# dyollb/segmantic

Hardware: AMD Instinct MI355X
Metric: 3D UNet train voxels/s on 128^3 bf16 (higher is better)
Workload: dtype bf16

## Files before the change

segmantic_amd/csrc/conv_fwd_impl.h:

```cpp
#pragma once
#include "common.h"
#include "fin_tail.h"

namespace segmi {

struct ConvParams {
  const void* in;
  void* out;
  const void* wfrag;
  const float* bias;
  const float* alpha;
  const void* res;
  float* stats;
  int N, Di, Hi, Wi, Do, Ho, Wo, Cin, Cout, ldi, ldo, ldr;
  int tz, ty, tx;
  int nchunks, ntiles_total;
  const float* in_scale;
  const float* in_shift;
  const float* in_alpha;
  int act_tiles;
  int stats_tiles;
  const float* bias2;
  const void* bx;
  int ldbx;
  const float* bmean; const float* binvstd; const float* bgamma; const float* bbeta; const float* balpha;
  float* bpart;
  int fin_on;
  FinTail ft;
  BnFin bfin;
  BnBwdFin bbfin;
  int xcd;
};

template <typename T, int CK, int KS, int S, int TD, int TH, int TW>
struct ConvGeom {
  static constexpr int KG = Elem<T>::KG;
  static constexpr int SPT = CK / KG;
  static constexpr int NTAPS = KS * KS * KS;
  static constexpr int NSLOT = NTAPS * SPT;
  static constexpr int NSTEP = (NSLOT + 3) / 4;
  static constexpr int PAD = (KS - 1) / 2;
  static constexpr int HD = (TD - 1) * S + KS;
  static constexpr int HH = (TH - 1) * S + KS;
  static constexpr int HW = (TW - 1) * S + KS;
  static constexpr int RAWB = CK * (int)sizeof(T);
  static constexpr int ROWB = RAWB == 32 ? 32 : RAWB + 16;
  static constexpr int CPR = RAWB / 16;
  static constexpr int NVT = TD * TH * TW / 16;
  static constexpr int VTW = NVT / 4;
  static constexpr int LDS_BYTES = HD * HH * HW * ROWB;
  static_assert(NVT % 4 == 0, "tile must give each wave whole voxel tiles");
  static_assert(SPT == 2 || SPT == 4 || SPT == 8, "unsupported chunk width");
};

template <typename T, int CK, int KS, int S, int NT, int TD, int TH, int TW>
__global__ __launch_bounds__(256) void conv_fwd_mfma_kernel(ConvParams p) {
  using G = ConvGeom<T, CK, KS, S, TD, TH, TW>;
  extern __shared__ __attribute__((aligned(16))) char smem[];
  const int tid = threadIdx.x, lane = tid & 63, wave = tid >> 6;
  const int g = lane >> 4, r = lane & 15;

  int t = blockIdx.x;
  const int txi = t % p.tx; t /= p.tx;
  const int tyi = t % p.ty; t /= p.ty;
  const int tzi = t % p.tz;
  const int n = t / p.tz;
  const int oz0 = tzi * TD, oy0 = tyi * TH, ox0 = txi * TW;
  const int iz0 = oz0 * S - G::PAD, iy0 = oy0 * S - G::PAD, ix0 = ox0 * S - G::PAD;
  const int nt0 = blockIdx.y * NT;

  f32x4 acc[G::VTW][NT];
#pragma unroll
  for (int i = 0; i < G::VTW; ++i)
#pragma unroll
    for (int j = 0; j < NT; ++j) acc[i][j] = f32x4{0.f, 0.f, 0.f, 0.f};

  int vaddr[G::VTW];
#pragma unroll
  for (int i = 0; i < G::VTW; ++i) {
    const int idx = (wave * G::VTW + i) * 16 + r;
    const int x = idx % TW, y = (idx / TW) % TH, z = idx / (TW * TH);
    vaddr[i] = ((z * S * G::HH + y * S) * G::HW + x * S) * G::ROWB;
  }

  constexpr bool PRE = G::NSTEP * NT <= 16;
  constexpr int WD = NT <= 2 ? (G::NSTEP < 4 ? G::NSTEP : 4) : 2;
  constexpr int NCH = G::HD * G::HH * G::HW * G::CPR;
  constexpr int NLD = (NCH + 255) / 256;
  constexpr bool PF = (G::VTW * NT * 4 + NLD * 4) <= 160;
  const char* inb = (const char*)p.in;
  frag_t stg[PF ? NLD : 1];
  auto fetch = [&](int c) {
#pragma unroll
    for (int k = 0; k < NLD; ++k) {
      const int i = tid + 256 * k;
      const int v = i / G::CPR, ch = i % G::CPR;
      const int hx = v % G::HW, hy = (v / G::HW) % G::HH, hz = v / (G::HW * G::HH);
      const int z = iz0 + hz, y = iy0 + hy, x = ix0 + hx;
      frag_t val = frag_t{0u, 0u, 0u, 0u};
      if (i < NCH && (unsigned)z < (unsigned)p.Di && (unsigned)y < (unsigned)p.Hi &&
          (unsigned)x < (unsigned)p.Wi) {
        const int64_t e = ((((int64_t)n * p.Di + z) * p.Hi + y) * p.Wi + x) * p.ldi + c * CK;
        val = *reinterpret_cast<const frag_t*>(inb + e * (int64_t)sizeof(T) + ch * 16);
      }
      if constexpr (PF) stg[k] = val;
      else if (i < NCH) *reinterpret_cast<frag_t*>(smem + v * G::ROWB + ch * 16) = val;
    }
  };
  if constexpr (PF) fetch(0);
  for (int c = 0; c < p.nchunks; ++c) {
    if (c > 0) __syncthreads();
    const char* wb = (const char*)p.wfrag +
                     (((int64_t)c * G::NSTEP) * p.ntiles_total + nt0) * 1024 + lane * 16;
    frag_t wall[PRE ? G::NSTEP : 1][NT];
    frag_t wq[PRE ? 1 : WD][NT];
    if constexpr (PRE) {
#pragma unroll
      for (int s = 0; s < G::NSTEP; ++s)
#pragma unroll
        for (int j = 0; j < NT; ++j)
          wall[s][j] = *reinterpret_cast<const frag_t*>(wb + ((int64_t)s * p.ntiles_total + j) * 1024);
    } else {
#pragma unroll
      for (int s = 0; s < WD; ++s)
#pragma unroll
        for (int j = 0; j < NT; ++j)
          wq[s][j] = *reinterpret_cast<const frag_t*>(wb + ((int64_t)s * p.ntiles_total + j) * 1024);
    }
    if constexpr (PF) {
#pragma unroll
      for (int k = 0; k < NLD; ++k) {
        const int i = tid + 256 * k;
        if (i < NCH) *reinterpret_cast<frag_t*>(smem + (i / G::CPR) * G::ROWB + (i % G::CPR) * 16) = stg[k];
      }
    } else {
      fetch(c);
    }
    __syncthreads();
    if constexpr (PF) {
      if (c + 1 < p.nchunks) fetch(c + 1);
    }
#pragma unroll
    for (int s = 0; s < G::NSTEP; ++s) {
      int loff;
      if constexpr (G::SPT == 2) {
        const int t0 = 2 * s, t1 = 2 * s + 1;
        const int o0 = ((t0 / (KS * KS)) * G::HH + (t0 / KS) % KS) * G::HW + t0 % KS;
        const int o1 = t1 < G::NTAPS
                           ? ((t1 / (KS * KS)) * G::HH + (t1 / KS) % KS) * G::HW + t1 % KS
                           : 0;
        loff = ((g >> 1) ? o1 : o0) * G::ROWB + (g & 1) * 16;
      } else {
        const int tap = (4 * s) / G::SPT;
        const int sub0 = (4 * s) % G::SPT;
        const int o0 = ((tap / (KS * KS)) * G::HH + (tap / KS) % KS) * G::HW + tap % KS;
        loff = o0 * G::ROWB + (sub0 + g) * 16;
      }
      frag_t wf[NT];
      if constexpr (PRE) {
#pragma unroll
        for (int j = 0; j < NT; ++j) wf[j] = wall[s][j];
      } else {
#pragma unroll
        for (int j = 0; j < NT; ++j) wf[j] = wq[s % WD][j];
        if (s + WD < G::NSTEP) {
#pragma unroll
          for (int j = 0; j < NT; ++j)
            wq[s % WD][j] = *reinterpret_cast<const frag_t*>(
                wb + ((int64_t)(s + WD) * p.ntiles_total + j) * 1024);
        }
      }
#pragma unroll
      for (int i = 0; i < G::VTW; ++i) {
        const frag_t a = *reinterpret_cast<const frag_t*>(smem + vaddr[i] + loff);
#pragma unroll
        for (int j = 0; j < NT; ++j) acc[i][j] = mma16<T>(wf[j], a, acc[i][j]);
      }
    }
  }

  f32x4 bias4[NT];
#pragma unroll
  for (int j = 0; j < NT; ++j) {
    bias4[j] = f32x4{0.f, 0.f, 0.f, 0.f};
    if (p.bias2 && nt0 + j >= p.act_tiles)
      bias4[j] = *reinterpret_cast<const f32x4*>(p.bias2 + (nt0 + j - p.act_tiles) * 16 + 4 * g);
    else if (p.bias) bias4[j] = *reinterpret_cast<const f32x4*>(p.bias + (nt0 + j) * 16 + 4 * g);
  }
  const bool has_alpha = p.alpha != nullptr;
  const float alpha = has_alpha ? *p.alpha : 0.f;
  const bool do_stats = p.stats != nullptr && (p.stats_tiles == 0 || nt0 < p.stats_tiles);
  const int stats_c = p.stats_tiles > 0 ? 16 * p.stats_tiles : p.Cout;
  f32x4 ssum[NT], ssq[NT];
#pragma unroll
  for (int j = 0; j < NT; ++j) {
    ssum[j] = f32x4{0.f, 0.f, 0.f, 0.f};
    ssq[j] = f32x4{0.f, 0.f, 0.f, 0.f};
  }
  T* outp = (T*)p.out;
  const T* resp = (const T*)p.res;
  f32x4 resv[G::VTW][NT];
  if (resp) {
#pragma unroll
    for (int i = 0; i < G::VTW; ++i) {
      const int idx = (wave * G::VTW + i) * 16 + r;
      const int oz = oz0 + idx / (TW * TH), oy = oy0 + (idx / TW) % TH, ox = ox0 + idx % TW;
      const bool valid = oz < p.Do && oy < p.Ho && ox < p.Wo;
      const int64_t vox = (((int64_t)n * p.Do + oz) * p.Ho + oy) * p.Wo + ox;
#pragma unroll
      for (int j = 0; j < NT; ++j)
        resv[i][j] = valid ? load4<T>(resp + vox * p.ldr + (nt0 + j) * 16 + 4 * g)
                           : f32x4{0.f, 0.f, 0.f, 0.f};
    }
#pragma unroll
    for (int i = 0; i < G::VTW; ++i)
#pragma unroll
      for (int j = 0; j < NT; ++j) touch_v(resv[i][j]);
  }
#pragma unroll
  for (int j = 0; j < NT; ++j) touch_v(bias4[j]);
  if constexpr (PF) {
#pragma unroll
    for (int k = 0; k < NLD; ++k) touch_v(stg[k]);
  }
#pragma unroll
  for (int i = 0; i < G::VTW; ++i) {
    const int idx = (wave * G::VTW + i) * 16 + r;
    const int oz = oz0 + idx / (TW * TH), oy = oy0 + (idx / TW) % TH, ox = ox0 + idx % TW;
    const bool valid = oz < p.Do && oy < p.Ho && ox < p.Wo;
    const int64_t vox = (((int64_t)n * p.Do + oz) * p.Ho + oy) * p.Wo + ox;
#pragma unroll
    for (int j = 0; j < NT; ++j) {
      f32x4 v = acc[i][j] + bias4[j];
      if (valid) {
        if (do_stats && (p.stats_tiles == 0 || nt0 + j < p.stats_tiles)) {
          ssum[j] += v;
          ssq[j] += v * v;
        }
        if (has_alpha && (p.act_tiles == 0 || nt0 + j < p.act_tiles)) {
#pragma unroll
          for (int e = 0; e < 4; ++e) v[e] = v[e] > 0.f ? v[e] : alpha * v[e];
        }
        const int co = (nt0 + j) * 16 + 4 * g;
        if (resp) v += resv[i][j];
        store4<T>(outp + vox * p.ldo + co, v);
      }
    }
  }
  if (do_stats) {
    __syncthreads();
    float* red = reinterpret_cast<float*>(smem);
#pragma unroll
    for (int j = 0; j < NT; ++j)
#pragma unroll
      for (int e = 0; e < 4; ++e) {
        const float a = row16_sum(ssum[j][e]);
        const float b = row16_sum(ssq[j][e]);
        if (r == 0) {
          red[(wave * 2 + 0) * NT * 16 + j * 16 + 4 * g + e] = a;
          red[(wave * 2 + 1) * NT * 16 + j * 16 + 4 * g + e] = b;
        }
      }
    __syncthreads();
    if (tid < 2 * NT * 16) {
      const int which = tid / (NT * 16), ch = tid % (NT * 16);
      float sacc = 0.f;
#pragma unroll
      for (int w = 0; w < 4; ++w) sacc += red[(w * 2 + which) * NT * 16 + ch];
      if (nt0 * 16 + ch < stats_c)
        fin_store(&p.stats[((int64_t)blockIdx.x * 2 + which) * stats_c + nt0 * 16 + ch], sacc);
    }
    fin_tail_run<BnFin, 256, offsetof(ConvParams, ft), offsetof(ConvParams, bfin)>(p.stats, smem);
  }
}

template <typename T, int CK, int KS, int S, int NT, int TD, int TH, int TW>
static int launch_conv_cfg(ConvParams p, hipStream_t st) {
  using G = ConvGeom<T, CK, KS, S, TD, TH, TW>;
  p.tz = cdiv(p.Do, TD);
  p.ty = cdiv(p.Ho, TH);
  p.tx = cdiv(p.Wo, TW);
  const int64_t nb = (int64_t)p.N * p.tz * p.ty * p.tx;
  SEGMI_CHECK_ARG(nb < (1ll << 31), "conv3d: too many tiles");
  dim3 grid((unsigned)nb, (unsigned)(p.Cout / (16 * NT)));
  constexpr int lds0 = G::LDS_BYTES > 4 * 2 * NT * 16 * 4 ? G::LDS_BYTES : 4 * 2 * NT * 16 * 4;
  p.fin_on = p.fin_on && p.stats;
  const int stats_c = p.stats_tiles > 0 ? 16 * p.stats_tiles : p.Cout;
  const dim3 sgrid(grid.x, (unsigned)cdiv(stats_c / 16, NT));
  const int lds = (int)fin_tail_arm(p, sgrid, 256, 2 * stats_c, lds0);
  auto kern = conv_fwd_mfma_kernel<T, CK, KS, S, NT, TD, TH, TW>;
  static bool attr_done = false;
  if (!attr_done && lds > 64 * 1024) {
    (void)hipFuncSetAttribute(reinterpret_cast<const void*>(kern),
                        hipFuncAttributeMaxDynamicSharedMemorySize, lds);
    attr_done = true;
  }
  hipLaunchKernelGGL(kern, grid, 256, lds, st, p);
  SEGMI_LAUNCH_CHECK("conv3d_fwd(mfma)");
  return SEGMI_OK;
}

template <typename T, int CK, int KS, int S, int NT>
static int launch_conv_tiles(const ConvParams& p, hipStream_t st) {
  const bool wide = p.Wo > 8;
  if constexpr (S == 1) {
    if (wide) return launch_conv_cfg<T, CK, KS, S, NT, 4, 8, 16>(p, st);
    return launch_conv_cfg<T, CK, KS, S, NT, 4, 4, 8>(p, st);
  } else {
    if (wide) return launch_conv_cfg<T, CK, KS, S, NT, 2, 4, 16>(p, st);
    return launch_conv_cfg<T, CK, KS, S, NT, 2, 4, 8>(p, st);
  }
}

template <typename T, int CK, int KS, int S>
static int launch_conv_nt(const ConvParams& p, hipStream_t st) {
  const int nt = p.Cout / 16;
  const bool wide = p.Wo > 8;
  const int td = S == 1 ? 4 : 2, th = S == 1 ? (wide ? 8 : 4) : 4, tw = wide ? 16 : 8;
  const int64_t tiles = (int64_t)p.N * cdiv(p.Do, td) * cdiv(p.Ho, th) * cdiv(p.Wo, tw);
  int sel = nt % 4 == 0 ? 4 : (nt % 2 == 0 ? 2 : 1);
  while (sel > 1 && tiles * (nt / sel) < 512) sel /= 2;
  if (sel == 4) return launch_conv_tiles<T, CK, KS, S, 4>(p, st);
  if (sel == 2) return launch_conv_tiles<T, CK, KS, S, 2>(p, st);
  return launch_conv_tiles<T, CK, KS, S, 1>(p, st);
}

template <typename T>
static int launch_conv_mfma_t(const ConvParams& p, int ksize, int stride, hipStream_t st) {
  constexpr int dt = DtypeOf<T>::value;
  const int ck = pick_ck(dt, p.Cin);
  if constexpr (sizeof(T) == 2) {
    if (ck == 32) {
      if (ksize == 3 && stride == 1) return launch_conv_nt<T, 32, 3, 1>(p, st);
      if (ksize == 3 && stride == 2) return launch_conv_nt<T, 32, 3, 2>(p, st);
      if (ksize == 1 && stride == 1) return launch_conv_nt<T, 32, 1, 1>(p, st);
    }
  }
  if (ksize == 3 && stride == 1) return launch_conv_nt<T, 16, 3, 1>(p, st);
  if (ksize == 3 && stride == 2) return launch_conv_nt<T, 16, 3, 2>(p, st);
  if (ksize == 1 && stride == 1) return launch_conv_nt<T, 16, 1, 1>(p, st);
  SEGMI_UNSUPPORTED("conv3d: unsupported ksize/stride %d/%d", ksize, stride);
}

static inline int conv_mfma_rows(const segmi_act* out, int stride) {
  const bool wide = out->w > 8;
  int td, th, tw;
  if (stride == 1) { td = 4; th = wide ? 8 : 4; tw = wide ? 16 : 8; }
  else { td = 2; th = 4; tw = wide ? 16 : 8; }
  return out->n * cdiv(out->d, td) * cdiv(out->h, th) * cdiv(out->w, tw);
}

}
```

segmantic_amd/csrc/conv_ks_impl.h:

```cpp
#pragma once
#include "conv_fwd_impl.h"

namespace segmi {

template <typename T, int CK, int KS, int S, int NT, int TD, int TH, int TW>
__global__ __launch_bounds__(256) void conv_fwd_ks_kernel(ConvParams p) {
  using G = ConvGeom<T, CK, KS, S, TD, TH, TW>;
  static_assert(G::SPT == 4, "k-split kernel: one k-step per tap");
  static_assert(G::NVT == 8, "k-split kernel: 8 voxel tiles per workgroup");
  constexpr int NSW = (G::NSTEP + 3) / 4;
  extern __shared__ __attribute__((aligned(16))) char smem[];
  const int tid = threadIdx.x, lane = tid & 63;
  const int wave = __builtin_amdgcn_readfirstlane(tid >> 6);
  const int g = lane >> 4, r = lane & 15;

  int t = blockIdx.x;
  const int txi = t % p.tx; t /= p.tx;
  const int tyi = t % p.ty; t /= p.ty;
  const int tzi = t % p.tz;
  const int n = t / p.tz;
  const int oz0 = tzi * TD, oy0 = tyi * TH, ox0 = txi * TW;
  const int iz0 = oz0 * S - G::PAD, iy0 = oy0 * S - G::PAD, ix0 = ox0 * S - G::PAD;
  const int nt0 = blockIdx.y * NT;

  f32x4 acc[8][NT];
#pragma unroll
  for (int i = 0; i < 8; ++i)
#pragma unroll
    for (int j = 0; j < NT; ++j) acc[i][j] = f32x4{0.f, 0.f, 0.f, 0.f};

  int vaddr[8];
#pragma unroll
  for (int i = 0; i < 8; ++i) {
    const int idx = i * 16 + r;
    const int x = idx % TW, y = (idx / TW) % TH, z = idx / (TW * TH);
    vaddr[i] = ((z * S * G::HH + y * S) * G::HW + x * S) * G::ROWB + g * 16;
  }
  int tapoff[NSW];
#pragma unroll
  for (int si = 0; si < NSW; ++si) {
    int tap = wave + 4 * si;
    if (tap > G::NTAPS - 1) tap = G::NTAPS - 1;
    tapoff[si] = (((tap / (KS * KS)) * G::HH + (tap / KS) % KS) * G::HW + tap % KS) * G::ROWB;
  }

  constexpr int NCH = G::HD * G::HH * G::HW * G::CPR;
  constexpr int NLD = (NCH + 255) / 256;
  const char* inb = (const char*)p.in;
  frag_t stg[NLD];
  auto fetch = [&](int c) {
#pragma unroll
    for (int k = 0; k < NLD; ++k) {
      const int i = tid + 256 * k;
      const int v = i / G::CPR, ch = i % G::CPR;
      const int hx = v % G::HW, hy = (v / G::HW) % G::HH, hz = v / (G::HW * G::HH);
      const int z = iz0 + hz, y = iy0 + hy, x = ix0 + hx;
      stg[k] = frag_t{0u, 0u, 0u, 0u};
      if (i < NCH && (unsigned)z < (unsigned)p.Di && (unsigned)y < (unsigned)p.Hi &&
          (unsigned)x < (unsigned)p.Wi) {
        const int64_t e = ((((int64_t)n * p.Di + z) * p.Hi + y) * p.Wi + x) * p.ldi + c * CK;
        stg[k] = *reinterpret_cast<const frag_t*>(inb + e * (int64_t)sizeof(T) + ch * 16);
      }
    }
  };
  const char* wb0 = (const char*)p.wfrag + (int64_t)nt0 * 1024 + lane * 16;
  frag_t wcur[NSW][NT], wnxt[NSW][NT];
  auto fetch_w = [&](int c, frag_t (&dst)[NSW][NT]) {
#pragma unroll
    for (int si = 0; si < NSW; ++si) {
      int s = wave + 4 * si;
      if (s > G::NSTEP - 1) s = G::NSTEP - 1;
#pragma unroll
      for (int j = 0; j < NT; ++j)
        dst[si][j] = *reinterpret_cast<const frag_t*>(
            wb0 + (((int64_t)c * G::NSTEP + s) * p.ntiles_total + j) * 1024);
    }
  };
  fetch(0);
  fetch_w(0, wcur);
  for (int c = 0; c < p.nchunks; ++c) {
    if (c > 0) __syncthreads();
#pragma unroll
    for (int k = 0; k < NLD; ++k) {
      const int i = tid + 256 * k;
      if (i < NCH) *reinterpret_cast<frag_t*>(smem + (i / G::CPR) * G::ROWB + (i % G::CPR) * 16) = stg[k];
    }
    __syncthreads();
    if (c + 1 < p.nchunks) {
      fetch(c + 1);
      fetch_w(c + 1, wnxt);
    }
#pragma unroll
    for (int si = 0; si < NSW; ++si) {
      const int s = wave + 4 * si;
      if (s < G::NSTEP) {
#pragma unroll
        for (int i = 0; i < 8; ++i) {
          const frag_t a = *reinterpret_cast<const frag_t*>(smem + vaddr[i] + tapoff[si]);
#pragma unroll
          for (int j = 0; j < NT; ++j) acc[i][j] = mma16<T>(wcur[si][j], a, acc[i][j]);
        }
      }
    }
#pragma unroll
    for (int si = 0; si < NSW; ++si)
#pragma unroll
      for (int j = 0; j < NT; ++j) wcur[si][j] = wnxt[si][j];
  }

  __syncthreads();
  f32x4* red = reinterpret_cast<f32x4*>(smem);
#pragma unroll
  for (int i = 0; i < 8; ++i)
#pragma unroll
    for (int j = 0; j < NT; ++j) red[((wave * 8 + i) * NT + j) * 64 + lane] = acc[i][j];
  __syncthreads();
  f32x4 fin[2][NT];
#pragma unroll
  for (int ii = 0; ii < 2; ++ii)
#pragma unroll
    for (int j = 0; j < NT; ++j) {
      const int i = wave * 2 + ii;
      f32x4 v = red[((0 * 8 + i) * NT + j) * 64 + lane];
      v += red[((1 * 8 + i) * NT + j) * 64 + lane];
      v += red[((2 * 8 + i) * NT + j) * 64 + lane];
      v += red[((3 * 8 + i) * NT + j) * 64 + lane];
      fin[ii][j] = v;
    }

  f32x4 bias4[NT];
#pragma unroll
  for (int j = 0; j < NT; ++j) {
    bias4[j] = f32x4{0.f, 0.f, 0.f, 0.f};
    if (p.bias) bias4[j] = *reinterpret_cast<const f32x4*>(p.bias + (nt0 + j) * 16 + 4 * g);
  }
  const bool has_alpha = p.alpha != nullptr;
  const float alpha = has_alpha ? *p.alpha : 0.f;
  f32x4 ssum[NT], ssq[NT];
#pragma unroll
  for (int j = 0; j < NT; ++j) {
    ssum[j] = f32x4{0.f, 0.f, 0.f, 0.f};
    ssq[j] = f32x4{0.f, 0.f, 0.f, 0.f};
  }
  T* outp = (T*)p.out;
  const T* resp = (const T*)p.res;
  f32x4 resv[2][NT];
  if (resp) {
#pragma unroll
    for (int ii = 0; ii < 2; ++ii) {
      const int idx = (wave * 2 + ii) * 16 + r;
      const int oz = oz0 + idx / (TW * TH), oy = oy0 + (idx / TW) % TH, ox = ox0 + idx % TW;
      const bool valid = oz < p.Do && oy < p.Ho && ox < p.Wo;
      const int64_t vox = (((int64_t)n * p.Do + oz) * p.Ho + oy) * p.Wo + ox;
#pragma unroll
      for (int j = 0; j < NT; ++j)
        resv[ii][j] = valid ? load4<T>(resp + vox * p.ldr + (nt0 + j) * 16 + 4 * g)
                            : f32x4{0.f, 0.f, 0.f, 0.f};
    }
#pragma unroll
    for (int ii = 0; ii < 2; ++ii)
#pragma unroll
      for (int j = 0; j < NT; ++j) touch_v(resv[ii][j]);
  }
#pragma unroll
  for (int j = 0; j < NT; ++j) touch_v(bias4[j]);
#pragma unroll
  for (int k = 0; k < NLD; ++k) touch_v(stg[k]);
#pragma unroll
  for (int ii = 0; ii < 2; ++ii) {
    const int idx = (wave * 2 + ii) * 16 + r;
    const int oz = oz0 + idx / (TW * TH), oy = oy0 + (idx / TW) % TH, ox = ox0 + idx % TW;
    const bool valid = oz < p.Do && oy < p.Ho && ox < p.Wo;
    const int64_t vox = (((int64_t)n * p.Do + oz) * p.Ho + oy) * p.Wo + ox;
#pragma unroll
    for (int j = 0; j < NT; ++j) {
      f32x4 v = fin[ii][j] + bias4[j];
      if (valid) {
        if (p.stats) {
          ssum[j] += v;
          ssq[j] += v * v;
        }
        if (has_alpha) {
#pragma unroll
          for (int e = 0; e < 4; ++e) v[e] = v[e] > 0.f ? v[e] : alpha * v[e];
        }
        const int co = (nt0 + j) * 16 + 4 * g;
        if (resp) v += resv[ii][j];
        store4<T>(outp + vox * p.ldo + co, v);
      }
    }
  }
  if (p.stats) {
    __syncthreads();
    float* rs = reinterpret_cast<float*>(smem);
#pragma unroll
    for (int j = 0; j < NT; ++j)
#pragma unroll
      for (int e = 0; e < 4; ++e) {
        const float a = row16_sum(ssum[j][e]);
        const float b = row16_sum(ssq[j][e]);
        if (r == 0) {
          rs[(wave * 2 + 0) * NT * 16 + j * 16 + 4 * g + e] = a;
          rs[(wave * 2 + 1) * NT * 16 + j * 16 + 4 * g + e] = b;
        }
      }
    __syncthreads();
    if (tid < 2 * NT * 16) {
      const int which = tid / (NT * 16), ch = tid % (NT * 16);
      float sacc = 0.f;
#pragma unroll
      for (int w = 0; w < 4; ++w) sacc += rs[(w * 2 + which) * NT * 16 + ch];
      fin_store(&p.stats[((int64_t)blockIdx.x * 2 + which) * p.Cout + nt0 * 16 + ch], sacc);
    }
    fin_tail_run<BnFin, 256, offsetof(ConvParams, ft), offsetof(ConvParams, bfin)>(p.stats, smem);
  }
}

template <typename T, int CK, int KS, int S, int NT, int TD, int TH, int TW>
static int launch_conv_ks_cfg(ConvParams p, hipStream_t st) {
  using G = ConvGeom<T, CK, KS, S, TD, TH, TW>;
  p.tz = cdiv(p.Do, TD);
  p.ty = cdiv(p.Ho, TH);
  p.tx = cdiv(p.Wo, TW);
  const int64_t nb = (int64_t)p.N * p.tz * p.ty * p.tx;
  SEGMI_CHECK_ARG(nb < (1ll << 31), "conv3d: too many tiles");
  dim3 grid((unsigned)nb, (unsigned)(p.Cout / (16 * NT)));
  constexpr int red = 4 * 8 * NT * 64 * 16;
  constexpr int lds0 = G::LDS_BYTES > red ? G::LDS_BYTES : red;
  p.fin_on = p.fin_on && p.stats;
  const int lds = (int)fin_tail_arm(p, grid, 256, 2 * p.Cout, lds0);
  auto kern = conv_fwd_ks_kernel<T, CK, KS, S, NT, TD, TH, TW>;
  static bool attr_done = false;
  if (!attr_done && lds > 64 * 1024) {
    (void)hipFuncSetAttribute(reinterpret_cast<const void*>(kern),
                              hipFuncAttributeMaxDynamicSharedMemorySize, lds);
    attr_done = true;
  }
  hipLaunchKernelGGL(kern, grid, 256, lds, st, p);
  SEGMI_LAUNCH_CHECK("conv3d_fwd(mfma, k-split)");
  return SEGMI_OK;
}

static inline int conv_ks_rows(const segmi_act* out) {
  const bool wide = out->w > 8;
  const int td = wide ? 2 : 4, th = 4, tw = wide ? 16 : 8;
  return out->n * cdiv(out->d, td) * cdiv(out->h, th) * cdiv(out->w, tw);
}
static inline bool conv_ks_ok(int dtype, int cin, int ksize, int stride) {
  if (ksize != 3 || stride != 1) return false;
  const int ck = pick_ck(dtype, cin);
  const int spt = ck / (dtype == SEGMI_F32 ? 4 : 8);
  return spt == 4 && cin >= ck;
}

template <typename T, int CK>
static int launch_conv_ks_t(const ConvParams& p, hipStream_t st) {
  const segmi_act o{nullptr, p.N, p.Do, p.Ho, p.Wo, p.Cout, p.Cout};
  const int nt = p.Cout / 16;
  const bool two = nt % 2 == 0 && (int64_t)conv_ks_rows(&o) * (nt / 2) >= 512;
  const bool wide = p.Wo > 8;
  if (two) return wide ? launch_conv_ks_cfg<T, CK, 3, 1, 2, 2, 4, 16>(p, st)
                       : launch_conv_ks_cfg<T, CK, 3, 1, 2, 4, 4, 8>(p, st);
  return wide ? launch_conv_ks_cfg<T, CK, 3, 1, 1, 2, 4, 16>(p, st)
              : launch_conv_ks_cfg<T, CK, 3, 1, 1, 4, 4, 8>(p, st);
}

}
```

Measured before the change: 3.584 billion.

## Make single-chunk k-split conv persistent with weight reuse and cross-tile prefetch

```diff
diff --git a/segmantic_amd/csrc/conv_fwd_impl.h b/segmantic_amd/csrc/conv_fwd_impl.h
--- a/segmantic_amd/csrc/conv_fwd_impl.h
+++ b/segmantic_amd/csrc/conv_fwd_impl.h
@@ -30,6 +30,7 @@
   BnFin bfin;
   BnBwdFin bbfin;
   int xcd;
+  int ntile, ntile_step;
 };
 
 template <typename T, int CK, int KS, int S, int TD, int TH, int TW>
diff --git a/segmantic_amd/csrc/conv_ks_impl.h b/segmantic_amd/csrc/conv_ks_impl.h
--- a/segmantic_amd/csrc/conv_ks_impl.h
+++ b/segmantic_amd/csrc/conv_ks_impl.h
@@ -1,10 +1,14 @@
 #pragma once
+#include <map>
+#include <mutex>
+#include <utility>
+
 #include "conv_fwd_impl.h"
 
 namespace segmi {
 
-template <typename T, int CK, int KS, int S, int NT, int TD, int TH, int TW>
-__global__ __launch_bounds__(256) void conv_fwd_ks_kernel(ConvParams p) {
+template <typename T, int CK, int KS, int S, int NT, int TD, int TH, int TW, bool WS>
+__global__ __launch_bounds__(256, 2) void conv_fwd_ks_kernel(ConvParams p) {
   using G = ConvGeom<T, CK, KS, S, TD, TH, TW>;
   static_assert(G::SPT == 4, "k-split kernel: one k-step per tap");
   static_assert(G::NVT == 8, "k-split kernel: 8 voxel tiles per workgroup");
@@ -13,21 +17,8 @@
   const int tid = threadIdx.x, lane = tid & 63;
   const int wave = __builtin_amdgcn_readfirstlane(tid >> 6);
   const int g = lane >> 4, r = lane & 15;
-
-  int t = blockIdx.x;
-  const int txi = t % p.tx; t /= p.tx;
-  const int tyi = t % p.ty; t /= p.ty;
-  const int tzi = t % p.tz;
-  const int n = t / p.tz;
-  const int oz0 = tzi * TD, oy0 = tyi * TH, ox0 = txi * TW;
-  const int iz0 = oz0 * S - G::PAD, iy0 = oy0 * S - G::PAD, ix0 = ox0 * S - G::PAD;
   const int nt0 = blockIdx.y * NT;
-
-  f32x4 acc[8][NT];
-#pragma unroll
-  for (int i = 0; i < 8; ++i)
-#pragma unroll
-    for (int j = 0; j < NT; ++j) acc[i][j] = f32x4{0.f, 0.f, 0.f, 0.f};
+  const int ntile = p.ntile, tstep = p.ntile_step;
 
   int vaddr[8];
 #pragma unroll
@@ -48,7 +39,13 @@
   constexpr int NLD = (NCH + 255) / 256;
   const char* inb = (const char*)p.in;
   frag_t stg[NLD];
-  auto fetch = [&](int c) {
+  auto fetch = [&](int tile, int c) {
+    int t = tile;
+    const int txi = t % p.tx; t /= p.tx;
+    const int tyi = t % p.ty; t /= p.ty;
+    const int tzi = t % p.tz;
+    const int n = t / p.tz;
+    const int iz0 = tzi * TD * S - G::PAD, iy0 = tyi * TH * S - G::PAD, ix0 = txi * TW * S - G::PAD;
 #pragma unroll
     for (int k = 0; k < NLD; ++k) {
       const int i = tid + 256 * k;
@@ -64,8 +61,8 @@
     }
   };
   const char* wb0 = (const char*)p.wfrag + (int64_t)nt0 * 1024 + lane * 16;
-  frag_t wcur[NSW][NT], wnxt[NSW][NT];
-  auto fetch_w = [&](int c, frag_t (&dst)[NSW][NT]) {
+  frag_t wcur[NSW][NT], wnxt[WS ? 1 : NSW][NT];
+  auto fetch_w = [&](int c, auto& dst) {
 #pragma unroll
     for (int si = 0; si < NSW; ++si) {
       int s = wave + 4 * si;
@@ -76,76 +73,121 @@
             wb0 + (((int64_t)c * G::NSTEP + s) * p.ntiles_total + j) * 1024);
     }
   };
-  fetch(0);
-  fetch_w(0, wcur);
-  for (int c = 0; c < p.nchunks; ++c) {
-    if (c > 0) __syncthreads();
-#pragma unroll
-    for (int k = 0; k < NLD; ++k) {
-      const int i = tid + 256 * k;
-      if (i < NCH) *reinterpret_cast<frag_t*>(smem + (i / G::CPR) * G::ROWB + (i % G::CPR) * 16) = stg[k];
-    }
-    __syncthreads();
-    if (c + 1 < p.nchunks) {
-      fetch(c + 1);
-      fetch_w(c + 1, wnxt);
-    }
-#pragma unroll
-    for (int si = 0; si < NSW; ++si) {
-      const int s = wave + 4 * si;
-      if (s < G::NSTEP) {
-#pragma unroll
-        for (int i = 0; i < 8; ++i) {
-          const frag_t a = *reinterpret_cast<const frag_t*>(smem + vaddr[i] + tapoff[si]);
-#pragma unroll
-          for (int j = 0; j < NT; ++j) acc[i][j] = mma16<T>(wcur[si][j], a, acc[i][j]);
-        }
-      }
-    }
-#pragma unroll
-    for (int si = 0; si < NSW; ++si)
-#pragma unroll
-      for (int j = 0; j < NT; ++j) wcur[si][j] = wnxt[si][j];
-  }
-
-  __syncthreads();
-  f32x4* red = reinterpret_cast<f32x4*>(smem);
-#pragma unroll
-  for (int i = 0; i < 8; ++i)
-#pragma unroll
-    for (int j = 0; j < NT; ++j) red[((wave * 8 + i) * NT + j) * 64 + lane] = acc[i][j];
-  __syncthreads();
-  f32x4 fin[2][NT];
-#pragma unroll
-  for (int ii = 0; ii < 2; ++ii)
-#pragma unroll
-    for (int j = 0; j < NT; ++j) {
-      const int i = wave * 2 + ii;
-      f32x4 v = red[((0 * 8 + i) * NT + j) * 64 + lane];
-      v += red[((1 * 8 + i) * NT + j) * 64 + lane];
-      v += red[((2 * 8 + i) * NT + j) * 64 + lane];
-      v += red[((3 * 8 + i) * NT + j) * 64 + lane];
-      fin[ii][j] = v;
-    }
-
-  f32x4 bias4[NT];
-#pragma unroll
-  for (int j = 0; j < NT; ++j) {
-    bias4[j] = f32x4{0.f, 0.f, 0.f, 0.f};
-    if (p.bias) bias4[j] = *reinterpret_cast<const f32x4*>(p.bias + (nt0 + j) * 16 + 4 * g);
-  }
   const bool has_alpha = p.alpha != nullptr;
   const float alpha = has_alpha ? *p.alpha : 0.f;
-  f32x4 ssum[NT], ssq[NT];
-#pragma unroll
-  for (int j = 0; j < NT; ++j) {
-    ssum[j] = f32x4{0.f, 0.f, 0.f, 0.f};
-    ssq[j] = f32x4{0.f, 0.f, 0.f, 0.f};
-  }
   T* outp = (T*)p.out;
   const T* resp = (const T*)p.res;
-  f32x4 resv[2][NT];
-  if (resp) {
+
+  const int nchunks = WS ? 1 : p.nchunks;
+  if constexpr (WS) {
+    fetch(blockIdx.x, 0);
+    fetch_w(0, wcur);
+  }
+  int tile = blockIdx.x;
+  do {
+    if constexpr (!WS) {
+      fetch(tile, 0);
+      fetch_w(0, wcur);
+    }
+    f32x4 acc[8][NT];
+#pragma unroll
+    for (int i = 0; i < 8; ++i)
+#pragma unroll
+      for (int j = 0; j < NT; ++j) acc[i][j] = f32x4{0.f, 0.f, 0.f, 0.f};
+
+    for (int c = 0; c < nchunks; ++c) {
+      __syncthreads();
+#pragma unroll
+      for (int k = 0; k < NLD; ++k) {
+        const int i = tid + 256 * k;
+        if (i < NCH) *reinterpret_cast<frag_t*>(smem + (i / G::CPR) * G::ROWB + (i % G::CPR) * 16) = stg[k];
+      }
+      __syncthreads();
+      if constexpr (WS) {
+        if (tile + tstep < ntile) fetch(tile + tstep, 0);
+      } else if (c + 1 < nchunks) {
+        fetch(tile, c + 1);
+        fetch_w(c + 1, wnxt);
+      }
+#pragma unroll
+      for (int si = 0; si < NSW; ++si) {
+        const int s = wave + 4 * si;
+        if (s < G::NSTEP) {
+#pragma unroll
+          for (int i = 0; i < 8; ++i) {
+            const frag_t a = *reinterpret_cast<const frag_t*>(smem + vaddr[i] + tapoff[si]);
+#pragma unroll
+            for (int j = 0; j < NT; ++j) acc[i][j] = mma16<T>(wcur[si][j], a, acc[i][j]);
+          }
+        }
+      }
+      if constexpr (!WS) {
+#pragma unroll
+        for (int si = 0; si < NSW; ++si)
+#pragma unroll
+          for (int j = 0; j < NT; ++j) wcur[si][j] = wnxt[si][j];
+      }
+    }
+
+    __syncthreads();
+    f32x4* red = reinterpret_cast<f32x4*>(smem);
+#pragma unroll
+    for (int i = 0; i < 8; ++i)
+#pragma unroll
+      for (int j = 0; j < NT; ++j) red[((wave * 8 + i) * NT + j) * 64 + lane] = acc[i][j];
+    __syncthreads();
+    f32x4 fin[2][NT];
+#pragma unroll
+    for (int ii = 0; ii < 2; ++ii)
+#pragma unroll
+      for (int j = 0; j < NT; ++j) {
+        const int i = wave * 2 + ii;
+        f32x4 v = red[((0 * 8 + i) * NT + j) * 64 + lane];
+        v += red[((1 * 8 + i) * NT + j) * 64 + lane];
+        v += red[((2 * 8 + i) * NT + j) * 64 + lane];
+        v += red[((3 * 8 + i) * NT + j) * 64 + lane];
+        fin[ii][j] = v;
+      }
+
+    int t = tile;
+    const int ox0 = (t % p.tx) * TW; t /= p.tx;
+    const int oy0 = (t % p.ty) * TH; t /= p.ty;
+    const int oz0 = (t % p.tz) * TD;
+    const int n = t / p.tz;
+    f32x4 bias4[NT];
+#pragma unroll
+    for (int j = 0; j < NT; ++j) {
+      bias4[j] = f32x4{0.f, 0.f, 0.f, 0.f};
+      if (p.bias) bias4[j] = *reinterpret_cast<const f32x4*>(p.bias + (nt0 + j) * 16 + 4 * g);
+    }
+    f32x4 ssum[NT], ssq[NT];
+#pragma unroll
+    for (int j = 0; j < NT; ++j) {
+      ssum[j] = f32x4{0.f, 0.f, 0.f, 0.f};
+      ssq[j] = f32x4{0.f, 0.f, 0.f, 0.f};
+    }
+    f32x4 resv[2][NT];
+    if (resp) {
+#pragma unroll
+      for (int ii = 0; ii < 2; ++ii) {
+        const int idx = (wave * 2 + ii) * 16 + r;
+        const int oz = oz0 + idx / (TW * TH), oy = oy0 + (idx / TW) % TH, ox = ox0 + idx % TW;
+        const bool valid = oz < p.Do && oy < p.Ho && ox < p.Wo;
+        const int64_t vox = (((int64_t)n * p.Do + oz) * p.Ho + oy) * p.Wo + ox;
+#pragma unroll
+        for (int j = 0; j < NT; ++j)
+          resv[ii][j] = valid ? load4<T>(resp + vox * p.ldr + (nt0 + j) * 16 + 4 * g)
+                              : f32x4{0.f, 0.f, 0.f, 0.f};
+      }
+#pragma unroll
+      for (int ii = 0; ii < 2; ++ii)
+#pragma unroll
+        for (int j = 0; j < NT; ++j) touch_v(resv[ii][j]);
+    }
+#pragma unroll
+    for (int j = 0; j < NT; ++j) touch_v(bias4[j]);
+#pragma unroll
+    for (int k = 0; k < NLD; ++k) touch_v(stg[k]);
 #pragma unroll
     for (int ii = 0; ii < 2; ++ii) {
       const int idx = (wave * 2 + ii) * 16 + r;
@@ -153,70 +195,76 @@
       const bool valid = oz < p.Do && oy < p.Ho && ox < p.Wo;
       const int64_t vox = (((int64_t)n * p.Do + oz) * p.Ho + oy) * p.Wo + ox;
 #pragma unroll
+      for (int j = 0; j < NT; ++j) {
+        f32x4 v = fin[ii][j] + bias4[j];
+        if (valid) {
+          if (p.stats) {
+            ssum[j] += v;
+            ssq[j] += v * v;
+          }
+          if (has_alpha) {
+#pragma unroll
+            for (int e = 0; e < 4; ++e) v[e] = v[e] > 0.f ? v[e] : alpha * v[e];
+          }
+          const int co = (nt0 + j) * 16 + 4 * g;
+          if (resp) v += resv[ii][j];
+          store4<T>(outp + vox * p.ldo + co, v);
+        }
+      }
+    }
+    if (p.stats) {
+      __syncthreads();
+      float* rs = reinterpret_cast<float*>(smem);
+#pragma unroll
       for (int j = 0; j < NT; ++j)
-        resv[ii][j] = valid ? load4<T>(resp + vox * p.ldr + (nt0 + j) * 16 + 4 * g)
-                            : f32x4{0.f, 0.f, 0.f, 0.f};
-    }
-#pragma unroll
-    for (int ii = 0; ii < 2; ++ii)
-#pragma unroll
-      for (int j = 0; j < NT; ++j) touch_v(resv[ii][j]);
-  }
-#pragma unroll
-  for (int j = 0; j < NT; ++j) touch_v(bias4[j]);
-#pragma unroll
-  for (int k = 0; k < NLD; ++k) touch_v(stg[k]);
-#pragma unroll
-  for (int ii = 0; ii < 2; ++ii) {
-    const int idx = (wave * 2 + ii) * 16 + r;
-    const int oz = oz0 + idx / (TW * TH), oy = oy0 + (idx / TW) % TH, ox = ox0 + idx % TW;
-    const bool valid = oz < p.Do && oy < p.Ho && ox < p.Wo;
-    const int64_t vox = (((int64_t)n * p.Do + oz) * p.Ho + oy) * p.Wo + ox;
-#pragma unroll
-    for (int j = 0; j < NT; ++j) {
-      f32x4 v = fin[ii][j] + bias4[j];
-      if (valid) {
-        if (p.stats) {
-          ssum[j] += v;
-          ssq[j] += v * v;
+#pragma unroll
+        for (int e = 0; e < 4; ++e) {
+          const float a = row16_sum(ssum[j][e]);
+          const float b = row16_sum(ssq[j][e]);
+          if (r == 0) {
+            rs[(wave * 2 + 0) * NT * 16 + j * 16 + 4 * g + e] = a;
+            rs[(wave * 2 + 1) * NT * 16 + j * 16 + 4 * g + e] = b;
+          }
         }
-        if (has_alpha) {
-#pragma unroll
-          for (int e = 0; e < 4; ++e) v[e] = v[e] > 0.f ? v[e] : alpha * v[e];
-        }
-        const int co = (nt0 + j) * 16 + 4 * g;
-        if (resp) v += resv[ii][j];
-        store4<T>(outp + vox * p.ldo + co, v);
-      }
-    }
-  }
+      __syncthreads();
+      if (tid < 2 * NT * 16) {
+        const int which = tid / (NT * 16), ch = tid % (NT * 16);
+        float sacc = 0.f;
+#pragma unroll
+        for (int w = 0; w < 4; ++w) sacc += rs[(w * 2 + which) * NT * 16 + ch];
+        fin_store(&p.stats[((int64_t)tile * 2 + which) * p.Cout + nt0 * 16 + ch], sacc);
+      }
+    }
+  } while (WS && (tile += tstep) < ntile);
   if (p.stats) {
-    __syncthreads();
-    float* rs = reinterpret_cast<float*>(smem);
-#pragma unroll
-    for (int j = 0; j < NT; ++j)
-#pragma unroll
-      for (int e = 0; e < 4; ++e) {
-        const float a = row16_sum(ssum[j][e]);
-        const float b = row16_sum(ssq[j][e]);
-        if (r == 0) {
-          rs[(wave * 2 + 0) * NT * 16 + j * 16 + 4 * g + e] = a;
-          rs[(wave * 2 + 1) * NT * 16 + j * 16 + 4 * g + e] = b;
-        }
-      }
-    __syncthreads();
-    if (tid < 2 * NT * 16) {
-      const int which = tid / (NT * 16), ch = tid % (NT * 16);
-      float sacc = 0.f;
-#pragma unroll
-      for (int w = 0; w < 4; ++w) sacc += rs[(w * 2 + which) * NT * 16 + ch];
-      fin_store(&p.stats[((int64_t)blockIdx.x * 2 + which) * p.Cout + nt0 * 16 + ch], sacc);
-    }
     fin_tail_run<BnFin, 256, offsetof(ConvParams, ft), offsetof(ConvParams, bfin)>(p.stats, smem);
   }
 }
 
-template <typename T, int CK, int KS, int S, int NT, int TD, int TH, int TW>
+template <typename T, int CK, int KS, int S, int NT, int TD, int TH, int TW, bool WS>
+static int conv_ks_capacity(int lds) {
+  static std::mutex mu;
+  static std::map<std::pair<int, int>, int> cache;
+  int dev = 0;
+  if (hipGetDevice(&dev) != hipSuccess) return 0;
+  std::lock_guard<std::mutex> lk(mu);
+  const auto key = std::make_pair(dev, lds);
+  auto it = cache.find(key);
+  if (it != cache.end()) return it->second;
+  int per_cu = 0, cus = 0;
+  auto kern = conv_fwd_ks_kernel<T, CK, KS, S, NT, TD, TH, TW, WS>;
+  if (lds > 64 * 1024)
+    (void)hipFuncSetAttribute(reinterpret_cast<const void*>(kern), hipFuncAttributeMaxDynamicSharedMemorySize, lds);
+  if (hipOccupancyMaxActiveBlocksPerMultiprocessor(&per_cu, reinterpret_cast<const void*>(kern), 256, lds) !=
+      hipSuccess)
+    per_cu = 0;
+  if (hipDeviceGetAttribute(&cus, hipDeviceAttributeMultiprocessorCount, dev) != hipSuccess) cus = 0;
+  (void)hipGetLastError();
+  cache[key] = per_cu * cus;
+  return per_cu * cus;
+}
+
+template <typename T, int CK, int KS, int S, int NT, int TD, int TH, int TW, bool WS>
 static int launch_conv_ks_cfg(ConvParams p, hipStream_t st) {
   using G = ConvGeom<T, CK, KS, S, TD, TH, TW>;
   p.tz = cdiv(p.Do, TD);
@@ -224,18 +272,30 @@
   p.tx = cdiv(p.Wo, TW);
   const int64_t nb = (int64_t)p.N * p.tz * p.ty * p.tx;
   SEGMI_CHECK_ARG(nb < (1ll << 31), "conv3d: too many tiles");
-  dim3 grid((unsigned)nb, (unsigned)(p.Cout / (16 * NT)));
+  p.ntile = (int)nb;
   constexpr int red = 4 * 8 * NT * 64 * 16;
   constexpr int lds0 = G::LDS_BYTES > red ? G::LDS_BYTES : red;
   p.fin_on = p.fin_on && p.stats;
-  const int lds = (int)fin_tail_arm(p, grid, 256, 2 * p.Cout, lds0);
-  auto kern = conv_fwd_ks_kernel<T, CK, KS, S, NT, TD, TH, TW>;
-  static bool attr_done = false;
-  if (!attr_done && lds > 64 * 1024) {
-    (void)hipFuncSetAttribute(reinterpret_cast<const void*>(kern),
-                              hipFuncAttributeMaxDynamicSharedMemorySize, lds);
-    attr_done = true;
-  }
+  size_t lds = lds0;
+  if (p.fin_on) {
+    const size_t need = fin_tail_lds(2 * p.Cout, 256);
+    if (need > lds) lds = need;
+  }
+  const unsigned gy = (unsigned)(p.Cout / (16 * NT));
+  const int cap = conv_ks_capacity<T, CK, KS, S, NT, TD, TH, TW, WS>((int)lds);
+  SEGMI_CHECK_ARG(cap > 0, "conv3d: the k-split kernel does not fit the device");
+  int64_t gx = nb;
+  if (WS) {
+    gx = cap / gy;
+    if (gx < 1) gx = 1;
+    if (gx > nb) gx = nb;
+    gx = cdiv64(nb, cdiv64(nb, gx));
+  }
+  dim3 grid((unsigned)gx, gy);
+  p.ntile_step = (int)gx;
+  if (p.fin_on) p.ft = fin_tail_make((int)nb, 2 * p.Cout, grid.x * grid.y);
+  else p.ft.on = 0;
+  auto kern = conv_fwd_ks_kernel<T, CK, KS, S, NT, TD, TH, TW, WS>;
   hipLaunchKernelGGL(kern, grid, 256, lds, st, p);
   SEGMI_LAUNCH_CHECK("conv3d_fwd(mfma, k-split)");
   return SEGMI_OK;
@@ -253,16 +313,21 @@
   return spt == 4 && cin >= ck;
 }
 
-template <typename T, int CK>
-static int launch_conv_ks_t(const ConvParams& p, hipStream_t st) {
+template <typename T, int CK, bool WS>
+static int launch_conv_ks_ws(const ConvParams& p, hipStream_t st) {
   const segmi_act o{nullptr, p.N, p.Do, p.Ho, p.Wo, p.Cout, p.Cout};
   const int nt = p.Cout / 16;
   const bool two = nt % 2 == 0 && (int64_t)conv_ks_rows(&o) * (nt / 2) >= 512;
   const bool wide = p.Wo > 8;
-  if (two) return wide ? launch_conv_ks_cfg<T, CK, 3, 1, 2, 2, 4, 16>(p, st)
-                       : launch_conv_ks_cfg<T, CK, 3, 1, 2, 4, 4, 8>(p, st);
-  return wide ? launch_conv_ks_cfg<T, CK, 3, 1, 1, 2, 4, 16>(p, st)
-              : launch_conv_ks_cfg<T, CK, 3, 1, 1, 4, 4, 8>(p, st);
-}
-
-}
+  if (two) return wide ? launch_conv_ks_cfg<T, CK, 3, 1, 2, 2, 4, 16, WS>(p, st)
+                       : launch_conv_ks_cfg<T, CK, 3, 1, 2, 4, 4, 8, WS>(p, st);
+  return wide ? launch_conv_ks_cfg<T, CK, 3, 1, 1, 2, 4, 16, WS>(p, st)
+              : launch_conv_ks_cfg<T, CK, 3, 1, 1, 4, 4, 8, WS>(p, st);
+}
+
+template <typename T, int CK>
+static int launch_conv_ks_t(const ConvParams& p, hipStream_t st) {
+  return p.nchunks == 1 ? launch_conv_ks_ws<T, CK, true>(p, st) : launch_conv_ks_ws<T, CK, false>(p, st);
+}
+
+}
```

Result: no change. 3.597 billion (median of 3 runs) (+0.3%).
